# Suaiba/Mammo-CLIP-Dissect

Measured on AMD Instinct MI355X. Metric: probe images/sec dissected (763 concepts, all layers), higher is better.
Workload: dtype f32; 1 GPU; configs[1]: M-Mammo-CLIP Dissect through the drop-in driver describe_broad_neurons.main(): Mammo-CLIP ViT-B/16 target+dissector (random init), weak: 10000 images per GPU, synthetic 224x224 images resident in HBM, 763 concepts, 12 layers x 768 neurons, soft_wpmi top_k=100; CSV + args.txt + activation cache files written inside the step; entry_point=mammo_clip_dissect_amd.concept_vit.describe_broad_neurons.main, images_per_gpu=10000, global_images=10000, batch=2500, parallelism=image-sharded dp1, activation_cache_written=True

## Files before the change

### mammo-clip-dissect_amd/_lib.py

```python
import ctypes
import os

_HERE = os.path.dirname(os.path.abspath(__file__))
LIB_PATH = os.environ.get("MCD_LIB_PATH") or os.path.join(_HERE, "csrc", "libmcd_hip.so")

_i64 = ctypes.c_int64
_int = ctypes.c_int
_f = ctypes.c_float
_p = ctypes.c_void_p
_sz = ctypes.c_size_t

SIGNATURES = {
    "mcd_last_error": (ctypes.c_char_p, []),
    "mcd_abi_version": (_int, []),
    "mcd_normalize_rows": (_int, [_p, _i64, _i64, _i64, _p, _i64, _p]),
    "mcd_center_cube_normalize_rows": (_int, [_p, _i64, _i64, _i64, _f, _p, _i64, _p]),
    "mcd_prepare_rows_gathered": (_int, [_p, _i64, _i64, _int, ctypes.POINTER(_i64), _i64, _i64, _i64, _int, _f, _p, _i64,
                                         _p]),
    "mcd_embed_gemm_workspace": (_sz, [_i64, _i64, _i64, _int]),
    "mcd_embed_gemm": (_int, [_p, _i64, _p, _i64, _i64, _i64, _i64, _int, _p, _i64, _p, _sz, _p]),
    "mcd_embed_gemm_exp_workspace": (_sz, [_i64, _i64, _i64]),
    "mcd_embed_gemm_exp": (_int, [_p, _i64, _p, _i64, _i64, _i64, _i64, _f, _int, _p, _i64, _p, _p, _sz, _p]),
    "mcd_embed_gemm_exp_time_kernel": (_int, [_int]),
    "mcd_embed_gemm_exp_kernel_ms": (_f, []),
# ... 22 lines not shown
    "mcd_conv7x7s2_nhwc": (_int, [_p, _i64, _i64, _i64, _i64, _p, _i64, _p, _p]),
    "mcd_bn_relu_maxpool_nhwc": (_int, [_p, _i64, _i64, _i64, _i64, _p, _p, _p, _p]),
    "mcd_conv_igemm_nhwc": (_int, [_p, _i64, _i64, _i64, _i64, _p, _p, _i64, _int, _int, _int, _int, _p, _p]),
    "mcd_conv_igemm_res_nhwc": (_int, [_p, _i64, _i64, _i64, _i64, _p, _p, _p, _i64, _int, _int, _int, _int, _p, _p]),
    "mcd_conv3x3s2_nhwc": (_int, [_p, _i64, _i64, _i64, _i64, _p, _p, _i64, _int, _p, _p]),
    "mcd_avgpool2_nhwc": (_int, [_p, _i64, _i64, _i64, _i64, _p, _p]),
    "mcd_attnpool_tokens": (_int, [_p, _i64, _i64, _i64, _p, _p, _p]),
    "mcd_image_preprocess": (_int, [_p, _i64, _i64, _i64, _p, _i64, _i64, _p, _i64, _i64, _i64, _i64, _i64, _i64, _p, _p, _i64,
                                    _p]),
    "mcd_image_minmax_workspace": (_sz, [_i64, _i64, _i64, _i64]),
    "mcd_image_minmax_normalize": (_int, [_p, _i64, _i64, _i64, _i64, _int, _f, _f, _p, _i64, _p, _sz, _p]),
}
TEXT_SIGNATURES = {
    "mcd_vit_attention_keylen": (_int, [_p, _i64, _i64, _i64, _p, _p, _p]),
    "mcd_text_embed_ln": (_int, [_p, _p, _p, _p, _p, _p, _p, _f, _i64, _i64, _i64, _i64, _i64, _p, _p]),
}
CLIP_SIGNATURES = {
    "mcd_vit_attention_causal": (_int, [_p, _i64, _i64, _i64, _p, _p]),
    "mcd_quick_gelu": (_int, [_p, _i64, _p, _p]),
}
TOKEN_SIGNATURES = {
    "mcd_token_mean": (_int, [_p, _int, _int, _int, _i64, _i64, _int, _p, _i64, _p]),
}

MCD_E_ARG = -1
MCD_E_RANGE = -2
MCD_E_WORKSPACE = -3
MCD_E_UNSUPPORTED = -5

_lib = None


class McdError(RuntimeError):

    def __init__(self, code, msg):
        super().__init__(msg)
        self.code = code


def load():
    global _lib
    if _lib is None:
        if not os.path.exists(LIB_PATH):
            raise ImportError(
                "mammo-clip-dissect_amd: %s not found. Build it with `python -c 'import __graft_entry__ as g; "
                "g.build()'` or `make -C mammo-clip-dissect_amd/csrc`. There is no CPU fallback." % LIB_PATH)
        L = ctypes.CDLL(LIB_PATH)
        for name, (res, args) in (list(SIGNATURES.items()) + list(TEXT_SIGNATURES.items()) + list(CLIP_SIGNATURES.items())
                                  + list(TOKEN_SIGNATURES.items())):
            fn = getattr(L, name)
            fn.restype = res
            fn.argtypes = args
        _lib = L
    return _lib


def check(rc):
    if rc != 0:
        msg = load().mcd_last_error().decode("utf-8", "replace")
        raise McdError(rc, msg)


BLASLT_PATH = os.path.join(os.path.dirname(LIB_PATH), "libmcd_blaslt.so")
BLASLT_SIGNATURES = {
    "mcd_blaslt_last_error": (ctypes.c_char_p, []),
    "mcd_linear_residual_workspace": (_sz, []),
    "mcd_linear_residual": (_int, [_p, _i64, _p, _i64, _p, _p, _i64, _p, _i64, _i64, _i64, _i64, _p, _sz, _p]),
    "mcd_linear_residual_relu": (_int, [_p, _i64, _p, _i64, _p, _p, _i64, _p, _i64, _i64, _i64, _i64, _p, _sz, _p]),
    "mcd_linear_residual_plan_info": (_int, [_i64, _i64, _i64, ctypes.POINTER(_f), ctypes.POINTER(_int)]),
    "mcd_linear_residual_get_picks": (_int, [ctypes.POINTER(_i64), _int]),
    "mcd_linear_residual_set_pick": (_int, [_i64, _i64, _i64, _int, _int]),
}
_blaslt = None


def load_blaslt():
    global _blaslt
    if _blaslt is None:
        try:
            L = ctypes.CDLL(BLASLT_PATH)
            for name, (res, args) in BLASLT_SIGNATURES.items():
                fn = getattr(L, name)
                fn.restype = res
                fn.argtypes = args
            _blaslt = L
        except (OSError, AttributeError):
            _blaslt = False
    return _blaslt or None
```

### mammo-clip-dissect_amd/concept_vit/utils.py

```python
import os
import re
import threading

import torch
from torch.utils.data import DataLoader

from .. import core
from ..pipeline import Dissector
from . import data_utils

PM_SUFFIX = {"max": "_max", "avg": ""}
_P_CACHE = {}


def get_activation(outputs, mode):
    if mode not in ("avg", "max"):
        raise ValueError("pool mode must be 'avg' or 'max'")

    def hook(model, input, output):
        if mode == 'avg' and type(output) is tuple:
            output = output[0]
        out = output.detach()
        if out.dim() not in (2, 3, 4):
            return
# ... 44 lines not shown
        words = (f.read()).split('\n')
    return [i for i in words if i != ""]


def _layer_widths(model, layers, sample, forward):
    cache = model.__dict__.setdefault("_mcd_layer_widths", {})
    missing = [m for m in layers if id(m) not in cache]
    if missing:
        got = {}
        hs = [m.register_forward_hook(lambda mod, i, o, k=id(m): got.__setitem__(k, o[0] if type(o) is tuple else o))
              for m in missing]
        with torch.no_grad():
            forward(sample)
        for h in hs:
            h.remove()
        for m in missing:
            o = got[id(m)]
            cache[id(m)] = int(o.shape[1] if o.dim() in (2, 4) else o.shape[2])
    return [cache[id(m)] for m in layers]


class Extraction:

    def __init__(self, dis, E_txt, target_layers, writer=None):
        self.dis, self.E_txt, self.target_layers, self.writer = dis, E_txt, list(target_layers), writer

    def start_writer(self):
        if self.writer is not None and not self.writer.is_alive() and not self.writer.started:
            self.writer.begin()

    def wait(self):
        if self.writer is not None:
            self.start_writer()
            self.writer.join()
            if self.writer.error is not None:
                raise self.writer.error
            self.writer = None


class _CacheWriter(threading.Thread):

    def __init__(self, device, jobs):
        super().__init__(daemon=True)
        self.device, self.jobs, self.error, self.started = device, jobs, None, False
        self.ready = None

    def begin(self):
        self.started = True
        if torch.device(self.device).type == "cuda":
            with torch.cuda.device(self.device):
                self.ready = torch.cuda.Event()
                self.ready.record()
        self.start()

    def _save_some(self, items):
        try:
            for t, path in items:
                torch.save(t, path)
        except Exception as e:
            self.error = e
# ... 59 lines not shown
            E_txt = torch.cat(feats)
            if write_caches:
                torch.save(E_txt.cpu(), text_save_name)
        if not (need_target or need_clip):
            return None
        if E_txt is None:
            E_txt = _load_feats(text_save_name, device)
        N = len(dataset)
        on_device = hasattr(dataset, "device_batches") and getattr(dataset, "device", None) is not None
        if on_device:
            batches = dataset.device_batches(batch_size)
            first = (dataset.sample() if hasattr(dataset, "sample") else dataset.images()[:1]) if N > 0 else None
        else:
            batches = DataLoader(dataset, batch_size=batch_size, shuffle=False, num_workers=0)
            first = _views(dataset[0][0])[0].unsqueeze(0).to(device) if N > 0 else None
        if first is None:
            first = torch.zeros((1, 3, 224, 224), dtype=torch.float32, device=device)
        layers = [resolve_layer(target_model, l) for l in target_layers]
        widths = _layer_widths(target_model, layers, first, encode_target)
        same = target_model is clip_model
        dis = Dissector(N, list(target_layers), widths, len(words), E_txt.shape[1], device,
                        pool_mode=pool_mode, gather=gather)
        handles = [m.register_forward_hook(dis.hook(i)) for i, m in enumerate(layers)] if need_target else []
        try:
            for batch in batches:
                if not on_device:
                    batch = batch[0] if isinstance(batch, (list, tuple)) else batch["images"]
                target_view, clip_view = _views(batch)
                images = target_view.to(device)
                clip_images = images if clip_view is target_view else clip_view.to(device)
                if need_target:
                    out = encode_target(images)
                if need_clip:
                    if same and need_target and clip_images is images:
                        f = out
                    else:
                        f = clip_model.encode_image(clip_images)
                    if getattr(clip_model, "projection", False):
                        f = clip_model.image_projection(f)
                    dis.add_image_features(f.float())
                dis.advance(images.shape[0])
        finally:
            for h in handles:
                h.remove()
        if not need_clip:
            dis.E_img.copy_(_load_feats(clip_save_name, device))
        if not need_target:
            for i, l in enumerate(target_layers):
                A = torch.load(layer_files[l], map_location='cpu', weights_only=True).float().to(device)
                core.transpose(A, out=dis.At[dis.offsets[i]:dis.offsets[i + 1], :N])
        writer = None
        if write_caches:
            jobs = []
            if need_clip:
                jobs.append((lambda: dis.E_img, clip_save_name))
            if need_target:
                for i, l in enumerate(target_layers):
                    jobs.append((lambda i=i: dis.At[dis.offsets[i]:dis.offsets[i + 1], :N].t(), layer_files[l]))
            writer = _CacheWriter(device, jobs)
        return Extraction(dis, E_txt, target_layers, writer)


def _views(batch):
    if isinstance(batch, (list, tuple)):
        target, clip = batch
        return target, clip
    return batch, batch


def _probe_data(d_probe, device, preprocess=None, clip_preprocess=None):
    from ..pipeline import shard_bounds
    world, rank = _dist_info()
    n = len(data_utils.get_data(d_probe, None))
    lo, hi = shard_bounds(n, world, rank)
# ... 65 lines not shown
```

### mammo-clip-dissect_amd/core.py

```python
import ctypes
import functools

import torch

from . import _lib
from ._lib import McdError, check

POOL_MODES = {"avg": 0, "max": 1, "cls": 2, "none": 3}
POOL_SILU_AVG = 4
GEMM_MODES = {"f32": 0, "bf16x3": 1, "bf16": 2}


def _stream():
    return ctypes.c_void_p(torch.cuda.current_stream().cuda_stream)


def _on_device(fn):
    @functools.wraps(fn)
    def wrapper(*args, **kw):
        dev = None
        for a in list(args) + list(kw.values()):
            if isinstance(a, torch.Tensor) and a.is_cuda:
                if dev is None:
                    dev = a.device
# ... 755 lines not shown
    if out is None:
        out = torch.empty(h.shape[:-1] + (N,), dtype=torch.float32, device=h.device)
    elif tuple(out.shape) != tuple(h.shape[:-1]) + (N,):
        raise ValueError("linear_residual: out has shape %s" % (tuple(out.shape),))
    ws = _blaslt_ws.get(h.device)
    if ws is None:
        ws = _blaslt_ws[h.device] = torch.empty((L.mcd_linear_residual_workspace(),), dtype=torch.uint8, device=h.device)
    ev = LINEAR_EVENTS
    if ev is not None:
        e0, e1 = torch.cuda.Event(enable_timing=True), torch.cuda.Event(enable_timing=True)
        e0.record()
    fn = L.mcd_linear_residual_relu if relu else L.mcd_linear_residual
    rc = fn(h.data_ptr(), ldh, weight.data_ptr(), K, bias.data_ptr() if bias is not None else None,
            res.data_ptr() if res is not None else None, ldr, out.data_ptr(), N, M, N, K, ws.data_ptr(), ws.numel(), _stream())
    if ev is not None:
        e1.record()
        ev.append((e0, e1, M, N, K))
    if rc != 0:
        raise _lib.McdError(rc, L.mcd_blaslt_last_error().decode("utf-8", "replace"))
    return out


@_on_device
def hook_pool(x, mode, dst, row0, col0, neuron_major):
    _need_gpu(x, dst)
    if x.dtype != torch.float32:
        x = x.float()
    nhwc = mode in ("avg", "max") and channels_last(x, only=True)
    if not nhwc:
        x = x.contiguous()
    if x.dim() == 4:
        B, Cout, HW = x.shape[0], x.shape[1], x.shape[2] * x.shape[3]
        m = POOL_MODES[mode]
    elif x.dim() == 3:
        B, HW, Cout = x.shape
        m = POOL_MODES["cls"]
    elif x.dim() == 2:
        B, Cout = x.shape
        HW = 1
        m = POOL_MODES["none"]
    else:
        raise ValueError("unsupported hook output shape %s" % (tuple(x.shape),))
    if dst.dtype != torch.float32 or dst.dim() != 2 or dst.stride(1) != 1:
        raise TypeError("dst must be a 2-D float32 matrix with unit inner stride")
    need = (col0 + Cout, row0 + B) if neuron_major else (row0 + B, col0 + Cout)
    if row0 < 0 or col0 < 0 or dst.shape[0] < need[0] or dst.shape[1] < need[1]:
        raise IndexError("hook_pool: block [%d:%d, %d:%d] outside the activation matrix %s"
                         % (row0, row0 + B, col0, col0 + Cout, tuple(dst.shape)))
    if neuron_major:
        sn, su = 1, dst.stride(0)
    else:
        sn, su = dst.stride(0), 1
    L = _lib.load()
    if nhwc:
        check(L.mcd_hook_pool_nhwc(x.data_ptr(), B, Cout, HW, m, dst.data_ptr(), int(row0), int(col0), sn, su, _stream()))
        return Cout
    check(L.mcd_hook_pool(x.data_ptr(), B, Cout, HW, m, dst.data_ptr(), int(row0), int(col0), sn, su, _stream()))
    return Cout


IMAGE_MAX_TAPS = 128
_PRECISION_BITS = 22
IMAGENET_MEAN, IMAGENET_STD = (0.485, 0.456, 0.406), (0.229, 0.224, 0.225)
CLIP_MEAN, CLIP_STD = (0.48145466, 0.4578275, 0.40821073), (0.26862954, 0.26130258, 0.27577711)


def _bilinear(x):
    x = -x if x < 0.0 else x
    return 1.0 - x if x < 1.0 else 0.0


def _bicubic(x):
    a = -0.5
    x = -x if x < 0.0 else x
    if x < 1.0:
        return ((a + 2.0) * x - (a + 3.0)) * x * x + 1
    if x < 2.0:
        return (((x - 5) * x + 8) * x - 4) * a
# ... 231 lines not shown
```

### mammo-clip-dissect_amd/csrc/k_pool.hip

```cpp
#include "mcd_common.h"

namespace {

template <bool VEC4>
__global__ __launch_bounds__(256) void pool_plane_kernel(const float* __restrict__ x, int64_t planes, int64_t Cout,
                                                          int64_t HW, int mode, float* __restrict__ dst, int64_t row0,
                                                          int64_t col0, int64_t stride_n, int64_t stride_u) {
    const int lane = threadIdx.x & 63;
    const int64_t plane = (int64_t)blockIdx.x * 4 + (threadIdx.x >> 6);
    if (plane >= planes) return;
    const float* src = x + plane * HW;
    float s = 0.f, m = -INFINITY;
    bool has_nan = false;
    if constexpr (VEC4) {
        const float4* s4 = reinterpret_cast<const float4*>(src);
        const int64_t n4 = HW >> 2;
        for (int64_t i = lane; i < n4; i += 64) {
            const float4 v = s4[i];
            s += (v.x + v.y) + (v.z + v.w);
            m = fmaxf(fmaxf(m, fmaxf(v.x, v.y)), fmaxf(v.z, v.w));
            has_nan |= (v.x != v.x) | (v.y != v.y) | (v.z != v.z) | (v.w != v.w);
        }
    } else {
        for (int64_t i = lane; i < HW; i += 64) {
            const float v = src[i];
            s += v;
            m = fmaxf(m, v);
            has_nan |= (v != v);
        }
    }
    s = mcd_wave_sum(s);
    m = mcd_wave_max(m);
    if (__ballot(has_nan)) m = __uint_as_float(0x7fc00000u);
    if (lane == 0) {
        const int64_t b = plane / Cout, ch = plane - b * Cout;
        dst[(row0 + b) * stride_n + (col0 + ch) * stride_u] = (mode == MCD_POOL_AVG) ? s / (float)HW : m;
    }
}

__global__ __launch_bounds__(256) void pool_copy_kernel(const float* __restrict__ x, int64_t B, int64_t F,
                                                         int64_t bstride, float* __restrict__ dst, int64_t row0,
                                                         int64_t col0, int64_t stride_n, int64_t stride_u) {
    const int64_t i = (int64_t)blockIdx.x * 256 + threadIdx.x;
    if (i >= B * F) return;
    const int64_t b = i / F, f = i - b * F;
    dst[(row0 + b) * stride_n + (col0 + f) * stride_u] = x[b * bstride + f];
}

}

extern "C" int mcd_hook_pool(const float* x, int64_t B, int64_t Cout, int64_t HW, int mode, float* dst, int64_t row0,
                             int64_t col0, int64_t stride_n, int64_t stride_u, mcd_stream_t stream) {
    MCD_REQUIRE(x && dst, MCD_E_ARG, "mcd_hook_pool: NULL pointer");
    MCD_REQUIRE(B >= 0 && Cout > 0 && HW > 0 && row0 >= 0 && col0 >= 0, MCD_E_ARG, "mcd_hook_pool: bad shape");
    MCD_REQUIRE(mode >= MCD_POOL_AVG && mode <= MCD_POOL_NONE, MCD_E_ARG, "mcd_hook_pool: bad mode %d", mode);
    if (B == 0) return MCD_OK;
    hipStream_t st = (hipStream_t)stream;
    if (mode == MCD_POOL_AVG || mode == MCD_POOL_MAX) {
        const int64_t planes = B * Cout;
        const unsigned grid = (unsigned)mcd_cdiv(planes, 4);
        const bool vec4 = (HW % 4 == 0) && (((uintptr_t)x) % 16 == 0);
        if (vec4)
            hipLaunchKernelGGL(pool_plane_kernel<true>, dim3(grid), dim3(256), 0, st, x, planes, Cout, HW, mode, dst,
                               row0, col0, stride_n, stride_u);
        else
            hipLaunchKernelGGL(pool_plane_kernel<false>, dim3(grid), dim3(256), 0, st, x, planes, Cout, HW, mode, dst,
                               row0, col0, stride_n, stride_u);
        MCD_LAUNCH_CHECK("pool_plane_kernel");
    } else {
        const int64_t bstride = (mode == MCD_POOL_CLS) ? HW * Cout : Cout;
        const unsigned grid = (unsigned)mcd_cdiv(B * Cout, 256);
        hipLaunchKernelGGL(pool_copy_kernel, dim3(grid), dim3(256), 0, st, x, B, Cout, bstride, dst, row0, col0,
                           stride_n, stride_u);
        MCD_LAUNCH_CHECK("pool_copy_kernel");
    }
    return MCD_OK;
}
```

### mammo-clip-dissect_amd/csrc/mcd_host.c

```c
#include <math.h>
#include <stdint.h>
#include <string.h>

static const double P10[9] = {1.0, 1e1, 1e2, 1e3, 1e4, 1e5, 1e6, 1e7, 1e8};
static const uint64_t I10[9] = {1ull, 10ull, 100ull, 1000ull, 10000ull, 100000ull, 1000000ull, 10000000ull, 100000000ull};

static int ndigits(uint64_t v) {
    int n = 1;
    while (v >= 10) { v /= 10; ++n; }
    return n;
}

static void shortest(float v, uint64_t* ip, uint64_t* fp, int* dp) {
    const float av = fabsf(v);
    const double x = (double)av;
    const double hi = (x + (double)nextafterf(av, INFINITY)) * 0.5, lo = (x + (double)nextafterf(av, 0.0f)) * 0.5;
    int d = 0, low = 0, high = 0;
    double y = 0, fl = 0;
    for (;; ++d) {
        y = x * P10[d];
        fl = floor(y);
        low = fl > lo * P10[d];
        high = fl + 1.0 < hi * P10[d];
        if (low || high || d == 8) break;
    }
// ... 142 lines not shown
            *e++ = '[';
            for (int j = 0; j < k; ++j) {
                const int32_t w = ids[r * k + j];
                if (w < 0 || w >= n_words) return -1;
                if (j) { *e++ = ','; *e++ = ' '; }
                memcpy(e, reprs[w], (size_t)repr_lens[w]);
                e += repr_lens[w];
            }
            *e++ = ']';
            o = emit_field(o, d, e - d);
        }
        *o++ = ',';
        int n = mcd_fmt_f32_row(vals + r * k, k, cell, (int)sizeof(cell));
        if (n < 0) return -1;
        o = emit_field(o, cell, n);
        *o++ = ',';
        n = mcd_fmt_i64_row(imgs + r * k_img, k_img, cell, (int)sizeof(cell));
        if (n < 0) return -1;
        o = emit_field(o, cell, n);
        *o++ = '\n';
    }
    return (int64_t)(o - out);
}
```

### mammo-clip-dissect_amd/pipeline.py

```python
import os

import torch
import torch.distributed as dist

from . import _lib
from . import core as _hip_ops


STAGE_MARK = None

ROW_FNS = ("rank_reorder", "cos_similarity", "cos_similarity_cubed")


def _round_up(x, m):
    return (x + m - 1) // m * m


def shard_align():
    try:
        return max(1, int(os.environ.get("MCD_SHARD_ALIGN", "1")))
    except ValueError:
        return 1


# ... 56 lines not shown
        if self.world > 1:
            mine = torch.tensor([[self.n_local]], dtype=torch.int64, device=self.device)
            self.counts = [int(v) for v in self._gather(mine).view(-1).tolist()]
        else:
            self.counts = [self.n_local]
        self.n_total = sum(self.counts)
        self.n_max = max(self.counts)
        self.row0 = sum(self.counts[:self.rank])
        self.layer_names = list(layer_names)
        self.layer_widths = [int(w) for w in layer_widths]
        self.offsets = [0]
        for w in self.layer_widths:
            self.offsets.append(self.offsets[-1] + w)
        self.U = self.offsets[-1]
        self.C, self.D = int(n_concepts), int(embed_dim)
        self.pool_mode = pool_mode
        self.gemm_mode = gemm_mode
        self.set_scoring(similarity_fn, None if similarity_fn in ROW_FNS else top_k, a=a, lam=lam, min_prob=min_prob,
                         p_start=p_start, p_end=p_end)
        self.ldA = _round_up(max(self.n_local, 1), 64)
        self.At = torch.zeros((self.U, self.ldA), dtype=torch.float32, device=self.device)
        self.E_img = torch.zeros((self.n_local, self.D), dtype=torch.float32, device=self.device)
        self.cursor = 0

    def set_scoring(self, similarity_fn="soft_wpmi", top_k=None, a=None, lam=None, min_prob=1e-7, p_start=0.998,
                    p_end=0.97, p=3, top_fraction=0.05, scale_p=0.5, min_norm=1e-3):
        if similarity_fn in ROW_FNS:
            if top_k is not None:
                raise TypeError("%s() got an unexpected keyword argument 'top_k'" % similarity_fn)
            if self.gemm_mode == "bf16":
                raise NotImplementedError("gemm_mode='bf16' never materialises fp32 P, which %s scores: use 'f32', "
                                          "'bf16x3' or 'bf16_p'" % similarity_fn)
            self.similarity_fn = similarity_fn
            self.top_k = 0
            self.rr_p, self.top_fraction, self.scale_p = float(p), float(top_fraction), float(scale_p)
            self.min_norm = float(min_norm)
            return
        if similarity_fn not in ("soft_wpmi", "wpmi"):
            raise NotImplementedError("fused pipeline supports soft_wpmi, wpmi, %s (got %r)" % (", ".join(ROW_FNS),
                                                                                             similarity_fn))
        self.similarity_fn = similarity_fn
        soft = similarity_fn == "soft_wpmi"
        self.top_k = int(top_k if top_k is not None else (100 if soft else 28))
        self.a = float(a if a is not None else (10 if soft else 2))
        self.lam = lam if lam is not None else (1 if soft else 0.6)
        self.min_prob = float(min_prob)
        self.p = None
        self.p_ok = True
        if soft:
            self.p = (p_start - (torch.arange(start=0, end=self.top_k) / self.top_k * (p_start - p_end))).float().to(
                self.device)
            self.p_ok = 0.0 <= min(p_start, p_end) and max(p_start, p_end) <= 1.0

    def reset(self):
        self.cursor = 0

    def hook(self, layer_index):
        col0 = self.offsets[layer_index]
        width = self.layer_widths[layer_index]

        def _hook(module, inputs, output):
            if type(output) is tuple:
                output = output[0]
            n = self.ops.hook_pool(output.detach(), self.pool_mode, self.At, self.cursor, col0, True)
            if n != width:
                raise RuntimeError("layer %s produced %d neurons, expected %d" % (self.layer_names[layer_index], n, width))
        _hook.token0_only = True
        return _hook

    def add_image_features(self, feats):
        B = feats.shape[0]
        self.E_img[self.cursor:self.cursor + B].copy_(feats)

    def advance(self, batch):
        self.cursor += int(batch)
        if self.cursor > self.n_local:
            raise RuntimeError("more images than the dissector was sized for")

    def _all_gather_rows(self, t):
        if self.world == 1:
            return t
        return self._gather(t.contiguous())

    def _all_gather_ragged(self, t, lens):
        if self.world == 1:
            return t[:lens[0]]
        m = max(lens)
        mine = lens[self.rank]
        if t.shape[0] != m:
            pad = torch.zeros((m,) + tuple(t.shape[1:]), dtype=t.dtype, device=t.device)
            pad[:mine] = t[:mine]
            t = pad
        full = self._gather(t.contiguous())
        if all(n == m for n in lens):
            return full
        return torch.cat([full[r * m:r * m + lens[r]] for r in range(self.world)], dim=0)

    def _col_topk_global(self, K, mark):
        ops, G, N_l = self.ops, self.world, self.n_local
        Kl = min(K, N_l)
# ... 397 lines not shown
```

Before: 3979 images/s.

## Stream activation cache rows to disk during extraction via pinned slots and host writer

Adds a cache-streaming path. The pooling hook also writes each batch's pooled rows into a row-major staging block, which is pushed through a slot ring to host code. That code writes the rows straight into a torch.save placeholder zip at the tensor record's offset, computes the CRC incrementally and patches it in at close. This is meant to remove the end-of-extraction transpose, torch.save and file write work by overlapping it with the forward passes. The cost is extra staging memory, per-batch reserve and push synchronisation, and reliance on the torch.save zip layout; it is limited to single-process runs.

```diff
diff --git a/include/mcd_cache.h b/include/mcd_cache.h
--- /dev/null
+++ b/include/mcd_cache.h
@@ -0,0 +1,43 @@
+#ifndef MCD_CACHE_H
+#define MCD_CACHE_H
+
+#include <stddef.h>
+#include <stdint.h>
+
+#include "mcd_hip.h"
+
+#ifdef __cplusplus
+extern "C" {
+#endif
+
+int mcd_hook_pool_rows(const float* x, int64_t B, int64_t Cout, int64_t HW, int mode, float* dst, int64_t row0,
+                       int64_t col0, int64_t stride_n, int64_t stride_u, float* rows, int64_t width,
+                       mcd_stream_t stream);
+
+typedef struct {
+    int (*append)(void* file, const float* rows, int64_t row0, int64_t n);
+    int (*close)(void* file);
+    void (*abort)(void* file);
+    const char* (*last_error)(void);
+} mcd_cache_io_t;
+
+int mcd_cache_stream_open(int n_files, void* const* files, const int64_t* widths, const mcd_cache_io_t* io, int n_slots,
+                          size_t slot_bytes, void** handle);
+int mcd_cache_stream_reserve(void* handle, int file, mcd_stream_t stream);
+int mcd_cache_stream_push(void* handle, int file, const float* device_block, int64_t row0, int64_t n,
+                          mcd_stream_t stream);
+int mcd_cache_stream_close(void* handle);
+int mcd_cache_stream_abort(void* handle);
+
+uint32_t mcd_zip_crc32(uint32_t crc, const void* buf, size_t n);
+int mcd_cachefile_open(const char* part_path, const char* final_path, int64_t n_rows, int64_t width, int64_t data_off,
+                       int64_t crc_off_a, int64_t crc_off_b, void** out);
+int mcd_cachefile_append(void* file, const float* rows, int64_t row0, int64_t n);
+int mcd_cachefile_close(void* file);
+void mcd_cachefile_abort(void* file);
+const char* mcd_cachefile_last_error(void);
+
+#ifdef __cplusplus
+}
+#endif
+#endif
diff --git a/mammo-clip-dissect_amd/_lib.py b/mammo-clip-dissect_amd/_lib.py
--- a/mammo-clip-dissect_amd/_lib.py
+++ b/mammo-clip-dissect_amd/_lib.py
@@ -68,6 +68,15 @@
 TOKEN_SIGNATURES = {
     "mcd_token_mean": (_int, [_p, _int, _int, _int, _i64, _i64, _int, _p, _i64, _p]),
 }
+_pp = ctypes.POINTER(_p)
+CACHE_SIGNATURES = {
+    "mcd_hook_pool_rows": (_int, [_p, _i64, _i64, _i64, _int, _p, _i64, _i64, _i64, _i64, _p, _i64, _p]),
+    "mcd_cache_stream_open": (_int, [_int, _pp, ctypes.POINTER(_i64), _p, _int, _sz, _pp]),
+    "mcd_cache_stream_reserve": (_int, [_p, _int, _p]),
+    "mcd_cache_stream_push": (_int, [_p, _int, _p, _i64, _i64, _p]),
+    "mcd_cache_stream_close": (_int, [_p]),
+    "mcd_cache_stream_abort": (_int, [_p]),
+}
 
 MCD_E_ARG = -1
 MCD_E_RANGE = -2
@@ -93,7 +102,7 @@
                 "g.build()'` or `make -C mammo-clip-dissect_amd/csrc`. There is no CPU fallback." % LIB_PATH)
         L = ctypes.CDLL(LIB_PATH)
         for name, (res, args) in (list(SIGNATURES.items()) + list(TEXT_SIGNATURES.items()) + list(CLIP_SIGNATURES.items())
-                                  + list(TOKEN_SIGNATURES.items())):
+                                  + list(TOKEN_SIGNATURES.items()) + list(CACHE_SIGNATURES.items())):
             fn = getattr(L, name)
             fn.restype = res
             fn.argtypes = args
@@ -133,3 +142,38 @@
         except (OSError, AttributeError):
             _blaslt = False
     return _blaslt or None
+
+
+HOST_PATH = os.path.join(_HERE, "csrc", "libmcd_host.so")
+CACHE_HOST_SIGNATURES = {
+    "mcd_zip_crc32": (ctypes.c_uint32, [ctypes.c_uint32, _p, _sz]),
+    "mcd_cachefile_open": (_int, [ctypes.c_char_p, ctypes.c_char_p, _i64, _i64, _i64, _i64, _i64, _pp]),
+    "mcd_cachefile_append": (_int, [_p, _p, _i64, _i64]),
+    "mcd_cachefile_close": (_int, [_p]),
+    "mcd_cachefile_abort": (None, [_p]),
+    "mcd_cachefile_last_error": (ctypes.c_char_p, []),
+}
+_cache_host = None
+
+
+class CacheIO(ctypes.Structure):
+    _fields_ = [("append", _p), ("close", _p), ("abort", _p), ("last_error", _p)]
+
+
+def load_cache_host():
+    global _cache_host
+    if _cache_host is None:
+        try:
+            L = ctypes.CDLL(HOST_PATH)
+            for name, (res, args) in CACHE_HOST_SIGNATURES.items():
+                fn = getattr(L, name)
+                fn.restype = res
+                fn.argtypes = args
+            _cache_host = L
+        except (OSError, AttributeError):
+            _cache_host = False
+    return _cache_host or None
+
+
+def cache_io(H):
+    return CacheIO(*[ctypes.cast(getattr(H, "mcd_cachefile_" + n), _p) for n in ("append", "close", "abort", "last_error")])
diff --git a/mammo-clip-dissect_amd/concept_vit/utils.py b/mammo-clip-dissect_amd/concept_vit/utils.py
--- a/mammo-clip-dissect_amd/concept_vit/utils.py
+++ b/mammo-clip-dissect_amd/concept_vit/utils.py
@@ -90,20 +90,170 @@
 
 class Extraction:
 
-    def __init__(self, dis, E_txt, target_layers, writer=None):
+    def __init__(self, dis, E_txt, target_layers, writer=None, stream=None):
         self.dis, self.E_txt, self.target_layers, self.writer = dis, E_txt, list(target_layers), writer
+        self.stream = stream
 
     def start_writer(self):
         if self.writer is not None and not self.writer.is_alive() and not self.writer.started:
             self.writer.begin()
 
     def wait(self):
+        if self.stream is not None:
+            stream, self.stream = self.stream, None
+            stream.close()
         if self.writer is not None:
             self.start_writer()
             self.writer.join()
             if self.writer.error is not None:
                 raise self.writer.error
             self.writer = None
+
+
+CACHE_STREAM_SLOTS = 8
+
+
+def _placeholder_archive(part_path, n_rows, width):
+    import struct
+    import zipfile
+    torch.save(torch.empty((n_rows, width), dtype=torch.float32), part_path)
+    nbytes = n_rows * width * 4
+    with zipfile.ZipFile(part_path) as z:
+        recs = [i for i in z.infolist() if i.filename.endswith("/data/0")]
+        start_dir = z.start_dir
+    with open(part_path, "rb") as f:
+        def at(off, n):
+            f.seek(off)
+            return f.read(n)
+        ok = len(recs) == 1 and recs[0].compress_type == zipfile.ZIP_STORED and recs[0].file_size == nbytes
+        if ok:
+            zi = recs[0]
+            head = at(zi.header_offset, 30)
+            ok = head[:4] == b"PK\x03\x04"
+        if ok:
+            n_name, n_extra = struct.unpack("<HH", head[26:30])
+            data_off = zi.header_offset + 30 + n_name + n_extra
+            if zi.flag_bits & 0x8:
+                crc_b = data_off + nbytes + (4 if at(data_off + nbytes, 4) == b"PK\x07\x08" else 0)
+            else:
+                crc_b = zi.header_offset + 14
+            crc_a, pos = None, start_dir
+            while crc_a is None:
+                ent = at(pos, 46)
+                if len(ent) < 46 or ent[:4] != b"PK\x01\x02":
+                    break
+                n_name, n_extra, n_comment = struct.unpack("<HHH", ent[28:34])
+                if at(pos + 46, n_name) == zi.orig_filename.encode("utf-8"):
+                    crc_a = pos + 16
+                pos += 46 + n_name + n_extra + n_comment
+            want = struct.pack("<I", zi.CRC)
+            ok = crc_a is not None and at(crc_a, 4) == want and at(crc_b, 4) == want
+    if not ok:
+        os.unlink(part_path)
+        raise RuntimeError("torch.save wrote an archive whose tensor record was not found where the zip format puts it: %s "
+                           "(MCD_CACHE_STREAM=0 writes the cache files without the streaming route)" % part_path)
+    return data_off, crc_a, crc_b
+
+
+class CacheStream:
+
+    def __init__(self, device, n_rows, files, batch_rows, slots=None):
+        d = torch.device(device)
+        self.device = torch.device("cuda", d.index if d.index is not None else torch.cuda.current_device())
+        self.n_rows, self.files = int(n_rows), list(files)
+        self.slots = int(slots if slots is not None else CACHE_STREAM_SLOTS)
+        self.slot_bytes = max(4, int(batch_rows) * max(w for _, w in self.files) * 4)
+        self.handle, self.pending, self.closed, self.keep = None, [], False, {}
+        self.L, self.H = core._lib.load(), core._lib.load_cache_host()
+
+    def begin(self):
+        if self.handle is not None or self.closed:
+            return
+        import ctypes
+        H, n = self.H, len(self.files)
+        handles = (ctypes.c_void_p * n)()
+        try:
+            for i, (path, width) in enumerate(self.files):
+                part = path + ".part"
+                data_off, crc_a, crc_b = _placeholder_archive(part, self.n_rows, width)
+                h = ctypes.c_void_p()
+                if H.mcd_cachefile_open(os.fsencode(part), os.fsencode(path), self.n_rows, width, data_off, crc_a, crc_b,
+                                        ctypes.byref(h)) != 0:
+                    raise OSError(H.mcd_cachefile_last_error().decode("utf-8", "replace"))
+                handles[i] = h
+        except BaseException:
+            self.closed = True
+            for h in handles:
+                if h:
+                    H.mcd_cachefile_abort(h)
+            raise
+        widths = (ctypes.c_int64 * n)(*[w for _, w in self.files])
+        io = core._lib.cache_io(H)
+        out = ctypes.c_void_p()
+        with torch.cuda.device(self.device):
+            rc = self.L.mcd_cache_stream_open(n, handles, widths, ctypes.byref(io), self.slots, self.slot_bytes, ctypes.byref(out))
+        if rc != 0:
+            self.closed = True
+            core.check(rc)
+        self.handle = out
+        pending, self.pending = self.pending, []
+        if pending:
+            with torch.cuda.device(self.device):
+                self._side = torch.cuda.Stream(device=self.device)
+                for file, block, row0, n, ready in pending:
+                    self._side.wait_event(ready)
+                    with torch.cuda.stream(self._side):
+                        self.push(file, block, row0, n)
+
+    def reserve(self, file):
+        if self.handle is not None:
+            with torch.cuda.device(self.device):
+                core.check(self.L.mcd_cache_stream_reserve(self.handle, file, core._stream()))
+
+    def push(self, file, block, row0, n):
+        if self.closed:
+            raise RuntimeError("CacheStream is closed")
+        if block.dtype != torch.float32 or not block.is_contiguous() or block.dim() != 2 or block.shape[0] < n \
+                or block.shape[1] != self.files[file][1] or block.device != self.device:
+            raise TypeError("CacheStream.push: block must be contiguous float32 [>= %d, %d] on %s" % (n, self.files[file][1], self.device))
+        if self.handle is None:
+            with torch.cuda.device(self.device):
+                ready = torch.cuda.Event()
+                ready.record()
+            self.pending.append((file, block, row0, n, ready))
+            return
+        self.keep[file] = block
+        with torch.cuda.device(self.device):
+            core.check(self.L.mcd_cache_stream_push(self.handle, file, block.data_ptr(), int(row0), int(n), core._stream()))
+
+    def _end(self, entry):
+        if self.closed:
+            return
+        self.closed = True
+        self.pending = []
+        if self.handle is not None:
+            handle, self.handle = self.handle, None
+            try:
+                core.check(entry(handle))
+            finally:
+                self.keep = {}
+
+    def close(self):
+        if not self.closed and self.handle is None:
+            self.begin()
+        self._end(self.L.mcd_cache_stream_close)
+
+    def abort(self):
+        try:
+            self._end(self.L.mcd_cache_stream_abort)
+        except core._lib.McdError:
+            pass
+
+    def __del__(self):
+        try:
+            self.abort()
+        except Exception:
+            pass
 
 
 class _CacheWriter(threading.Thread):
@@ -209,6 +359,14 @@
         dis = Dissector(N, list(target_layers), widths, len(words), E_txt.shape[1], device,
                         pool_mode=pool_mode, gather=gather)
         handles = [m.register_forward_hook(dis.hook(i)) for i, m in enumerate(layers)] if need_target else []
+        stream = None
+        if write_caches and need_target and N > 0 and torch.device(device).type == "cuda" \
+                and os.environ.get("MCD_CACHE_STREAM", "1") != "0" and core._lib.load_cache_host() is not None:
+            files = [(layer_files[l], w) for l, w in zip(target_layers, widths)]
+            if need_clip:
+                files.append((clip_save_name, int(E_txt.shape[1])))
+            stream = CacheStream(dis.device, N, files, batch_size)
+            dis.attach_cache_stream(stream, batch_size, image_file=len(files) - 1 if need_clip else None)
         try:
             for batch in batches:
                 if not on_device:
@@ -227,9 +385,14 @@
                         f = clip_model.image_projection(f)
                     dis.add_image_features(f.float())
                 dis.advance(images.shape[0])
+        except BaseException:
+            if stream is not None:
+                stream.abort()
+            raise
         finally:
             for h in handles:
                 h.remove()
+            dis.cache_stream = None
         if not need_clip:
             dis.E_img.copy_(_load_feats(clip_save_name, device))
         if not need_target:
@@ -237,6 +400,8 @@
                 A = torch.load(layer_files[l], map_location='cpu', weights_only=True).float().to(device)
                 core.transpose(A, out=dis.At[dis.offsets[i]:dis.offsets[i + 1], :N])
         writer = None
+        if stream is not None:
+            return Extraction(dis, E_txt, target_layers, stream=stream)
         if write_caches:
             jobs = []
             if need_clip:
diff --git a/mammo-clip-dissect_amd/core.py b/mammo-clip-dissect_amd/core.py
--- a/mammo-clip-dissect_amd/core.py
+++ b/mammo-clip-dissect_amd/core.py
@@ -801,8 +801,10 @@
 
 
 @_on_device
-def hook_pool(x, mode, dst, row0, col0, neuron_major):
+def hook_pool(x, mode, dst, row0, col0, neuron_major, rows=None):
     _need_gpu(x, dst)
+    if rows is not None:
+        _need_gpu(rows)
     if x.dtype != torch.float32:
         x = x.float()
     nhwc = mode in ("avg", "max") and channels_last(x, only=True)
@@ -830,9 +832,21 @@
         sn, su = 1, dst.stride(0)
     else:
         sn, su = dst.stride(0), 1
+    if rows is not None and (rows.dtype != torch.float32 or rows.dim() != 2 or not rows.is_contiguous()
+                             or rows.shape[0] < B or rows.shape[1] != Cout):
+        raise TypeError("rows must be a contiguous float32 [>= %d, %d] block" % (B, Cout))
     L = _lib.load()
     if nhwc:
         check(L.mcd_hook_pool_nhwc(x.data_ptr(), B, Cout, HW, m, dst.data_ptr(), int(row0), int(col0), sn, su, _stream()))
+        if rows is not None:
+            if not neuron_major:
+                raise TypeError("hook_pool: rows with a channels-last input needs a neuron-major dst")
+            if B > 0:
+                transpose(dst[col0:col0 + Cout, row0:row0 + B], out=rows[:B])
+        return Cout
+    if rows is not None:
+        check(L.mcd_hook_pool_rows(x.data_ptr(), B, Cout, HW, m, dst.data_ptr(), int(row0), int(col0), sn, su, rows.data_ptr(),
+                                   Cout, _stream()))
         return Cout
     check(L.mcd_hook_pool(x.data_ptr(), B, Cout, HW, m, dst.data_ptr(), int(row0), int(col0), sn, su, _stream()))
     return Cout
diff --git a/mammo-clip-dissect_amd/csrc/k_pool.hip b/mammo-clip-dissect_amd/csrc/k_pool.hip
--- a/mammo-clip-dissect_amd/csrc/k_pool.hip
+++ b/mammo-clip-dissect_amd/csrc/k_pool.hip
@@ -1,11 +1,13 @@
 #include "mcd_common.h"
+#include "../../include/mcd_cache.h"
 
 namespace {
 
-template <bool VEC4>
+template <bool VEC4, bool ROWS>
 __global__ __launch_bounds__(256) void pool_plane_kernel(const float* __restrict__ x, int64_t planes, int64_t Cout,
                                                           int64_t HW, int mode, float* __restrict__ dst, int64_t row0,
-                                                          int64_t col0, int64_t stride_n, int64_t stride_u) {
+                                                          int64_t col0, int64_t stride_n, int64_t stride_u,
+                                                          float* __restrict__ rows, int64_t width) {
     const int lane = threadIdx.x & 63;
     const int64_t plane = (int64_t)blockIdx.x * 4 + (threadIdx.x >> 6);
     if (plane >= planes) return;
@@ -34,26 +36,32 @@
     if (__ballot(has_nan)) m = __uint_as_float(0x7fc00000u);
     if (lane == 0) {
         const int64_t b = plane / Cout, ch = plane - b * Cout;
-        dst[(row0 + b) * stride_n + (col0 + ch) * stride_u] = (mode == MCD_POOL_AVG) ? s / (float)HW : m;
+        const float v = (mode == MCD_POOL_AVG) ? s / (float)HW : m;
+        dst[(row0 + b) * stride_n + (col0 + ch) * stride_u] = v;
+        if constexpr (ROWS) rows[b * width + ch] = v;
     }
 }
 
+template <bool ROWS>
 __global__ __launch_bounds__(256) void pool_copy_kernel(const float* __restrict__ x, int64_t B, int64_t F,
                                                          int64_t bstride, float* __restrict__ dst, int64_t row0,
-                                                         int64_t col0, int64_t stride_n, int64_t stride_u) {
+                                                         int64_t col0, int64_t stride_n, int64_t stride_u,
+                                                         float* __restrict__ rows, int64_t width) {
     const int64_t i = (int64_t)blockIdx.x * 256 + threadIdx.x;
     if (i >= B * F) return;
     const int64_t b = i / F, f = i - b * F;
-    dst[(row0 + b) * stride_n + (col0 + f) * stride_u] = x[b * bstride + f];
+    const float v = x[b * bstride + f];
+    dst[(row0 + b) * stride_n + (col0 + f) * stride_u] = v;
+    if constexpr (ROWS) rows[b * width + f] = v;
 }
 
-}
-
-extern "C" int mcd_hook_pool(const float* x, int64_t B, int64_t Cout, int64_t HW, int mode, float* dst, int64_t row0,
-                             int64_t col0, int64_t stride_n, int64_t stride_u, mcd_stream_t stream) {
-    MCD_REQUIRE(x && dst, MCD_E_ARG, "mcd_hook_pool: NULL pointer");
-    MCD_REQUIRE(B >= 0 && Cout > 0 && HW > 0 && row0 >= 0 && col0 >= 0, MCD_E_ARG, "mcd_hook_pool: bad shape");
-    MCD_REQUIRE(mode >= MCD_POOL_AVG && mode <= MCD_POOL_NONE, MCD_E_ARG, "mcd_hook_pool: bad mode %d", mode);
+template <bool ROWS>
+int hook_pool(const char* who, const float* x, int64_t B, int64_t Cout, int64_t HW, int mode, float* dst, int64_t row0,
+              int64_t col0, int64_t stride_n, int64_t stride_u, float* rows, int64_t width, mcd_stream_t stream) {
+    MCD_REQUIRE(x && dst, MCD_E_ARG, "%s: NULL pointer", who);
+    MCD_REQUIRE(B >= 0 && Cout > 0 && HW > 0 && row0 >= 0 && col0 >= 0, MCD_E_ARG, "%s: bad shape", who);
+    MCD_REQUIRE(mode >= MCD_POOL_AVG && mode <= MCD_POOL_NONE, MCD_E_ARG, "%s: bad mode %d", who, mode);
+    if (ROWS) MCD_REQUIRE(rows && width >= Cout, MCD_E_ARG, "%s: rows is NULL or width %lld < Cout", who, (long long)width);
     if (B == 0) return MCD_OK;
     hipStream_t st = (hipStream_t)stream;
     if (mode == MCD_POOL_AVG || mode == MCD_POOL_MAX) {
@@ -61,18 +69,31 @@
         const unsigned grid = (unsigned)mcd_cdiv(planes, 4);
         const bool vec4 = (HW % 4 == 0) && (((uintptr_t)x) % 16 == 0);
         if (vec4)
-            hipLaunchKernelGGL(pool_plane_kernel<true>, dim3(grid), dim3(256), 0, st, x, planes, Cout, HW, mode, dst,
-                               row0, col0, stride_n, stride_u);
+            hipLaunchKernelGGL((pool_plane_kernel<true, ROWS>), dim3(grid), dim3(256), 0, st, x, planes, Cout, HW, mode, dst,
+                               row0, col0, stride_n, stride_u, rows, width);
         else
-            hipLaunchKernelGGL(pool_plane_kernel<false>, dim3(grid), dim3(256), 0, st, x, planes, Cout, HW, mode, dst,
-                               row0, col0, stride_n, stride_u);
+            hipLaunchKernelGGL((pool_plane_kernel<false, ROWS>), dim3(grid), dim3(256), 0, st, x, planes, Cout, HW, mode, dst,
+                               row0, col0, stride_n, stride_u, rows, width);
         MCD_LAUNCH_CHECK("pool_plane_kernel");
     } else {
         const int64_t bstride = (mode == MCD_POOL_CLS) ? HW * Cout : Cout;
         const unsigned grid = (unsigned)mcd_cdiv(B * Cout, 256);
-        hipLaunchKernelGGL(pool_copy_kernel, dim3(grid), dim3(256), 0, st, x, B, Cout, bstride, dst, row0, col0,
-                           stride_n, stride_u);
+        hipLaunchKernelGGL(pool_copy_kernel<ROWS>, dim3(grid), dim3(256), 0, st, x, B, Cout, bstride, dst, row0, col0,
+                           stride_n, stride_u, rows, width);
         MCD_LAUNCH_CHECK("pool_copy_kernel");
     }
     return MCD_OK;
 }
+
+}
+
+extern "C" int mcd_hook_pool(const float* x, int64_t B, int64_t Cout, int64_t HW, int mode, float* dst, int64_t row0,
+                             int64_t col0, int64_t stride_n, int64_t stride_u, mcd_stream_t stream) {
+    return hook_pool<false>("mcd_hook_pool", x, B, Cout, HW, mode, dst, row0, col0, stride_n, stride_u, nullptr, 0, stream);
+}
+
+extern "C" int mcd_hook_pool_rows(const float* x, int64_t B, int64_t Cout, int64_t HW, int mode, float* dst, int64_t row0,
+                                  int64_t col0, int64_t stride_n, int64_t stride_u, float* rows, int64_t width,
+                                  mcd_stream_t stream) {
+    return hook_pool<true>("mcd_hook_pool_rows", x, B, Cout, HW, mode, dst, row0, col0, stride_n, stride_u, rows, width, stream);
+}
diff --git a/mammo-clip-dissect_amd/csrc/mcd_cache.hip b/mammo-clip-dissect_amd/csrc/mcd_cache.hip
--- /dev/null
+++ b/mammo-clip-dissect_amd/csrc/mcd_cache.hip
@@ -0,0 +1,255 @@
+#include <condition_variable>
+#include <deque>
+#include <mutex>
+#include <string>
+#include <thread>
+#include <vector>
+
+#include "mcd_common.h"
+#include "../../include/mcd_cache.h"
+
+namespace {
+
+struct Slot {
+    void* host = nullptr;
+    hipEvent_t done = nullptr;
+};
+
+struct Ring {
+    std::mutex mu;
+    std::vector<Slot> slots;
+    size_t slot_bytes = 0;
+    int device = -1;
+    bool lent = false;
+};
+Ring g_ring;
+
+struct Job {
+    int slot, file;
+    int64_t row0, n;
+};
+
+struct Writer {
+    int device = 0;
+    hipStream_t copy = nullptr;
+    hipEvent_t ready = nullptr;
+    std::vector<void*> files;
+    std::vector<int64_t> widths;
+    std::vector<hipEvent_t> file_done;
+    std::vector<char> file_pushed;
+    mcd_cache_io_t io{};
+    int n_slots = 0;
+    size_t slot_bytes = 0;
+
+    std::mutex mu;
+    std::condition_variable cv_job, cv_free;
+    std::deque<Job> jobs;
+    std::vector<int> free_slots;
+    bool stop = false;
+    int err = MCD_OK;
+    std::string err_text;
+    std::thread worker;
+
+    void fail(int code, const std::string& text) {
+        if (err == MCD_OK) {
+            err = code;
+            err_text = text;
+        }
+    }
+};
+
+void ring_release_storage(Ring& r) {
+    for (Slot& s : r.slots) {
+        if (s.done) (void)hipEventDestroy(s.done);
+        if (s.host) (void)hipHostFree(s.host);
+    }
+    r.slots.clear();
+    r.slot_bytes = 0;
+}
+
+int ring_borrow(int device, int n_slots, size_t slot_bytes) {
+    std::lock_guard<std::mutex> g(g_ring.mu);
+    MCD_REQUIRE(!g_ring.lent, MCD_E_UNSUPPORTED, "mcd_cache_stream_open: another stream writer of this process is still open");
+    if (g_ring.device != device || g_ring.slot_bytes < slot_bytes || (int)g_ring.slots.size() < n_slots) {
+        ring_release_storage(g_ring);
+        g_ring.device = device;
+        for (int i = 0; i < n_slots; ++i) {
+            Slot s;
+            hipError_t e = hipHostMalloc(&s.host, slot_bytes, hipHostMallocDefault);
+            if (e == hipSuccess) e = hipEventCreateWithFlags(&s.done, hipEventDisableTiming | hipEventBlockingSync);
+            if (e != hipSuccess) {
+                if (s.host) (void)hipHostFree(s.host);
+                ring_release_storage(g_ring);
+                return mcd_fail(MCD_E_LAUNCH, "mcd_cache_stream_open: pinned slot %d of %zu bytes: %s", i, slot_bytes, hipGetErrorString(e));
+            }
+            g_ring.slots.push_back(s);
+        }
+        g_ring.slot_bytes = slot_bytes;
+    }
+    g_ring.lent = true;
+    return MCD_OK;
+}
+
+void ring_return() {
+    std::lock_guard<std::mutex> g(g_ring.mu);
+    g_ring.lent = false;
+}
+
+void worker_main(Writer* w) {
+    (void)hipSetDevice(w->device);
+    for (;;) {
+        Job j;
+        {
+            std::unique_lock<std::mutex> lk(w->mu);
+            w->cv_job.wait(lk, [&] { return w->stop || !w->jobs.empty(); });
+            if (w->jobs.empty()) return;
+            j = w->jobs.front();
+            w->jobs.pop_front();
+        }
+        const Slot& s = g_ring.slots[(size_t)j.slot];
+        const hipError_t e = hipEventSynchronize(s.done);
+        bool ok;
+        {
+            std::lock_guard<std::mutex> g(w->mu);
+            if (e != hipSuccess) w->fail(MCD_E_LAUNCH, std::string("mcd_cache_stream: device -> host copy: ") + hipGetErrorString(e));
+            ok = w->err == MCD_OK;
+        }
+        if (ok && w->io.append(w->files[(size_t)j.file], (const float*)s.host, j.row0, j.n) != 0) {
+            const char* t = w->io.last_error ? w->io.last_error() : nullptr;
+            std::lock_guard<std::mutex> g(w->mu);
+            w->fail(MCD_E_UNSUPPORTED, std::string("mcd_cache_stream: append: ") + (t ? t : "failed"));
+        }
+        {
+            std::lock_guard<std::mutex> g(w->mu);
+            w->free_slots.push_back(j.slot);
+        }
+        w->cv_free.notify_one();
+    }
+}
+
+void writer_destroy(Writer* w) {
+    for (hipEvent_t e : w->file_done)
+        if (e) (void)hipEventDestroy(e);
+    if (w->ready) (void)hipEventDestroy(w->ready);
+    if (w->copy) (void)hipStreamDestroy(w->copy);
+    delete w;
+}
+
+int writer_end(void* handle, bool commit, const char* who) {
+    Writer* w = (Writer*)handle;
+    MCD_REQUIRE(w, MCD_E_ARG, "%s: NULL handle", who);
+    {
+        std::lock_guard<std::mutex> g(w->mu);
+        w->stop = true;
+    }
+    w->cv_job.notify_one();
+    if (w->worker.joinable()) w->worker.join();
+    ring_return();
+    for (void* f : w->files) {
+        if (commit && w->err == MCD_OK) {
+            if (w->io.close(f) != 0) {
+                const char* t = w->io.last_error ? w->io.last_error() : nullptr;
+                w->fail(MCD_E_UNSUPPORTED, std::string("mcd_cache_stream_close: ") + (t ? t : "finalisation failed"));
+            }
+        } else {
+            w->io.abort(f);
+        }
+    }
+    const int err = w->err;
+    const std::string text = w->err_text;
+    writer_destroy(w);
+    return err == MCD_OK ? MCD_OK : mcd_fail(err, "%s", text.c_str());
+}
+
+}
+
+extern "C" int mcd_cache_stream_open(int n_files, void* const* files, const int64_t* widths, const mcd_cache_io_t* io, int n_slots,
+                                     size_t slot_bytes, void** handle) {
+    MCD_REQUIRE(handle, MCD_E_ARG, "mcd_cache_stream_open: NULL handle pointer");
+    *handle = nullptr;
+    const bool io_ok = io && io->append && io->close && io->abort;
+    bool args_ok = io_ok && n_files >= 1 && files && widths && n_slots >= 1 && n_slots <= 1024 && slot_bytes >= 4;
+    for (int i = 0; args_ok && i < n_files; ++i) args_ok = files[i] != nullptr && widths[i] > 0;
+    if (!args_ok) {
+        if (io_ok && files)
+            for (int i = 0; i < n_files; ++i)
+                if (files[i]) io->abort(files[i]);
+        return mcd_fail(MCD_E_ARG, "mcd_cache_stream_open: bad argument");
+    }
+    Writer* w = new Writer;
+    w->files.assign(files, files + n_files);
+    w->widths.assign(widths, widths + n_files);
+    w->io = *io;
+    w->file_done.assign((size_t)n_files, nullptr);
+    w->file_pushed.assign((size_t)n_files, 0);
+    w->n_slots = n_slots;
+    w->slot_bytes = slot_bytes;
+    hipError_t e = hipGetDevice(&w->device);
+    if (e == hipSuccess) e = hipStreamCreateWithFlags(&w->copy, hipStreamNonBlocking);
+    if (e == hipSuccess) e = hipEventCreateWithFlags(&w->ready, hipEventDisableTiming);
+    for (int i = 0; e == hipSuccess && i < n_files; ++i) e = hipEventCreateWithFlags(&w->file_done[(size_t)i], hipEventDisableTiming);
+    int rc = e == hipSuccess ? MCD_OK : mcd_fail(MCD_E_LAUNCH, "mcd_cache_stream_open: %s", hipGetErrorString(e));
+    if (rc == MCD_OK) rc = ring_borrow(w->device, n_slots, slot_bytes);
+    if (rc != MCD_OK) {
+        for (void* f : w->files) w->io.abort(f);
+        writer_destroy(w);
+        return rc;
+    }
+    for (int i = 0; i < n_slots; ++i) w->free_slots.push_back(i);
+    w->worker = std::thread(worker_main, w);
+    *handle = w;
+    return MCD_OK;
+}
+
+extern "C" int mcd_cache_stream_reserve(void* handle, int file, mcd_stream_t stream) {
+    Writer* w = (Writer*)handle;
+    MCD_REQUIRE(w && file >= 0 && file < (int)w->files.size(), MCD_E_ARG, "mcd_cache_stream_reserve: bad handle or file %d", file);
+    if (!w->file_pushed[(size_t)file]) return MCD_OK;
+    const hipError_t e = hipStreamWaitEvent((hipStream_t)stream, w->file_done[(size_t)file], 0);
+    MCD_REQUIRE(e == hipSuccess, MCD_E_LAUNCH, "mcd_cache_stream_reserve: %s", hipGetErrorString(e));
+    return MCD_OK;
+}
+
+extern "C" int mcd_cache_stream_push(void* handle, int file, const float* device_block, int64_t row0, int64_t n,
+                                     mcd_stream_t stream) {
+    Writer* w = (Writer*)handle;
+    MCD_REQUIRE(w && file >= 0 && file < (int)w->files.size(), MCD_E_ARG, "mcd_cache_stream_push: bad handle or file %d", file);
+    MCD_REQUIRE(row0 >= 0 && n >= 0, MCD_E_ARG, "mcd_cache_stream_push: bad rows");
+    if (n == 0) return MCD_OK;
+    MCD_REQUIRE(device_block, MCD_E_ARG, "mcd_cache_stream_push: NULL block");
+    const int64_t width = w->widths[(size_t)file];
+    MCD_REQUIRE((uint64_t)n <= w->slot_bytes / 4 / (uint64_t)width, MCD_E_ARG,
+                "mcd_cache_stream_push: %lld rows of %lld floats do not fit a slot of %zu bytes", (long long)n, (long long)width, w->slot_bytes);
+    const size_t bytes = (size_t)n * (size_t)width * 4;
+    int slot;
+    {
+        std::unique_lock<std::mutex> lk(w->mu);
+        w->cv_free.wait(lk, [&] { return !w->free_slots.empty(); });
+        slot = w->free_slots.back();
+        w->free_slots.pop_back();
+    }
+    const Slot& s = g_ring.slots[(size_t)slot];
+    hipError_t e = hipEventRecord(w->ready, (hipStream_t)stream);
+    if (e == hipSuccess) e = hipStreamWaitEvent(w->copy, w->ready, 0);
+    if (e == hipSuccess) e = hipMemcpyAsync(s.host, device_block, bytes, hipMemcpyDeviceToHost, w->copy);
+    if (e == hipSuccess) e = hipEventRecord(s.done, w->copy);
+    if (e == hipSuccess) e = hipEventRecord(w->file_done[(size_t)file], w->copy);
+    if (e != hipSuccess) {
+        (void)hipStreamSynchronize(w->copy);
+        std::lock_guard<std::mutex> g(w->mu);
+        w->free_slots.push_back(slot);
+        w->fail(MCD_E_LAUNCH, std::string("mcd_cache_stream_push: ") + hipGetErrorString(e));
+        return mcd_fail(MCD_E_LAUNCH, "mcd_cache_stream_push: %s", hipGetErrorString(e));
+    }
+    w->file_pushed[(size_t)file] = 1;
+    {
+        std::lock_guard<std::mutex> g(w->mu);
+        w->jobs.push_back(Job{slot, file, row0, n});
+    }
+    w->cv_job.notify_one();
+    return MCD_OK;
+}
+
+extern "C" int mcd_cache_stream_close(void* handle) { return writer_end(handle, true, "mcd_cache_stream_close"); }
+
+extern "C" int mcd_cache_stream_abort(void* handle) { return writer_end(handle, false, "mcd_cache_stream_abort"); }
diff --git a/mammo-clip-dissect_amd/csrc/mcd_host.c b/mammo-clip-dissect_amd/csrc/mcd_host.c
--- a/mammo-clip-dissect_amd/csrc/mcd_host.c
+++ b/mammo-clip-dissect_amd/csrc/mcd_host.c
@@ -1,6 +1,12 @@
+#define _POSIX_C_SOURCE 200809L
+#include <errno.h>
+#include <fcntl.h>
 #include <math.h>
 #include <stdint.h>
+#include <stdio.h>
+#include <stdlib.h>
 #include <string.h>
+#include <unistd.h>
 
 static const double P10[9] = {1.0, 1e1, 1e2, 1e3, 1e4, 1e5, 1e6, 1e7, 1e8};
 static const uint64_t I10[9] = {1ull, 10ull, 100ull, 1000ull, 10000ull, 100000ull, 1000000ull, 10000000ull, 100000000ull};
@@ -189,3 +195,156 @@
     }
     return (int64_t)(o - out);
 }
+
+static _Thread_local char g_cache_err[512];
+
+const char* mcd_cachefile_last_error(void) { return g_cache_err; }
+
+static int cache_fail(const char* what, const char* path, int err) {
+    if (err)
+        snprintf(g_cache_err, sizeof g_cache_err, "%s: %s: %s", what, path ? path : "", strerror(err));
+    else
+        snprintf(g_cache_err, sizeof g_cache_err, "%s: %s", what, path ? path : "");
+    return -1;
+}
+
+static uint32_t g_crc_tab[8][256];
+static int g_crc_ready;
+
+static void crc_init(void) {
+    for (uint32_t i = 0; i < 256; ++i) {
+        uint32_t c = i;
+        for (int k = 0; k < 8; ++k) c = (c & 1u) ? 0xEDB88320u ^ (c >> 1) : c >> 1;
+        g_crc_tab[0][i] = c;
+    }
+    for (uint32_t i = 0; i < 256; ++i)
+        for (int t = 1; t < 8; ++t) g_crc_tab[t][i] = (g_crc_tab[t - 1][i] >> 8) ^ g_crc_tab[0][g_crc_tab[t - 1][i] & 0xffu];
+    __atomic_store_n(&g_crc_ready, 1, __ATOMIC_RELEASE);
+}
+
+uint32_t mcd_zip_crc32(uint32_t crc, const void* buf, size_t n) {
+    const unsigned char* p = (const unsigned char*)buf;
+    if (!__atomic_load_n(&g_crc_ready, __ATOMIC_ACQUIRE)) crc_init();
+    uint32_t c = ~crc;
+    while (n && ((uintptr_t)p & 7u)) { c = g_crc_tab[0][(c ^ *p++) & 0xffu] ^ (c >> 8); --n; }
+    while (n >= 8) {
+        uint32_t lo, hi;
+        memcpy(&lo, p, 4);
+        memcpy(&hi, p + 4, 4);
+        lo ^= c;
+        c = g_crc_tab[7][lo & 0xffu] ^ g_crc_tab[6][(lo >> 8) & 0xffu] ^ g_crc_tab[5][(lo >> 16) & 0xffu] ^ g_crc_tab[4][lo >> 24] ^
+            g_crc_tab[3][hi & 0xffu] ^ g_crc_tab[2][(hi >> 8) & 0xffu] ^ g_crc_tab[1][(hi >> 16) & 0xffu] ^ g_crc_tab[0][hi >> 24];
+        p += 8;
+        n -= 8;
+    }
+    while (n--) c = g_crc_tab[0][(c ^ *p++) & 0xffu] ^ (c >> 8);
+    return ~c;
+}
+
+typedef struct {
+    int fd;
+    int64_t n_rows, width, rows_done, data_off, crc_off[2];
+    uint32_t crc;
+    char *part, *final;
+} mcd_cachefile;
+
+static int write_all(int fd, const void* buf, size_t n, int64_t off) {
+    const char* p = (const char*)buf;
+    while (n) {
+        const ssize_t w = pwrite(fd, p, n, (off_t)off);
+        if (w < 0) {
+            if (errno == EINTR) continue;
+            return -1;
+        }
+        p += w;
+        off += w;
+        n -= (size_t)w;
+    }
+    return 0;
+}
+
+static void cachefile_drop(mcd_cachefile* f, int unlink_part) {
+    if (f->fd >= 0) close(f->fd);
+    if (unlink_part && f->part) unlink(f->part);
+    free(f->part);
+    free(f->final);
+    free(f);
+}
+
+int mcd_cachefile_open(const char* part_path, const char* final_path, int64_t n_rows, int64_t width, int64_t data_off,
+                       int64_t crc_off_a, int64_t crc_off_b, void** out) {
+    if (!part_path || !final_path || !out) return cache_fail("mcd_cachefile_open", "NULL argument", 0);
+    *out = NULL;
+    if (n_rows < 0 || width <= 0 || data_off < 0 || crc_off_a < 0 || crc_off_b < 0 || n_rows > (INT64_MAX >> 3) / width)
+        return cache_fail("mcd_cachefile_open: bad shape or offset", part_path, 0);
+    const int64_t bytes = n_rows * width * 4, end = data_off + bytes;
+    const int64_t c[2] = {crc_off_a, crc_off_b};
+    for (int i = 0; i < 2; ++i)
+        if (c[i] + 4 > data_off && c[i] < end)
+            return cache_fail("mcd_cachefile_open: a CRC field lies inside the data record", part_path, 0);
+    mcd_cachefile* f = (mcd_cachefile*)calloc(1, sizeof *f);
+    if (!f) return cache_fail("mcd_cachefile_open: out of memory", part_path, 0);
+    f->fd = -1;
+    f->part = strdup(part_path);
+    f->final = strdup(final_path);
+    if (!f->part || !f->final) {
+        cachefile_drop(f, 0);
+        return cache_fail("mcd_cachefile_open: out of memory", part_path, 0);
+    }
+    f->fd = open(part_path, O_WRONLY | O_CLOEXEC);
+    if (f->fd < 0) {
+        const int e = errno;
+        cachefile_drop(f, 0);
+        return cache_fail("mcd_cachefile_open", part_path, e);
+    }
+    const off_t size = lseek(f->fd, 0, SEEK_END);
+    if (size < 0 || (int64_t)size < end || (int64_t)size < crc_off_a + 4 || (int64_t)size < crc_off_b + 4) {
+        cachefile_drop(f, 1);
+        return cache_fail("mcd_cachefile_open: the placeholder archive is shorter than its record", part_path, 0);
+    }
+    f->n_rows = n_rows;
+    f->width = width;
+    f->data_off = data_off;
+    f->crc_off[0] = crc_off_a;
+    f->crc_off[1] = crc_off_b;
+    *out = f;
+    return 0;
+}
+
+int mcd_cachefile_append(void* h, const float* rows, int64_t row0, int64_t n) {
+    mcd_cachefile* f = (mcd_cachefile*)h;
+    if (!f || n < 0 || (n > 0 && !rows)) return cache_fail("mcd_cachefile_append", "bad argument", 0);
+    if (row0 != f->rows_done) return cache_fail("mcd_cachefile_append: rows out of order", f->part, 0);
+    if (n > f->n_rows - f->rows_done) return cache_fail("mcd_cachefile_append: more rows than the file was opened for", f->part, 0);
+    const size_t bytes = (size_t)n * (size_t)f->width * 4;
+    if (write_all(f->fd, rows, bytes, f->data_off + f->rows_done * f->width * 4) != 0) return cache_fail("mcd_cachefile_append", f->part, errno);
+    f->crc = mcd_zip_crc32(f->crc, rows, bytes);
+    f->rows_done += n;
+    return 0;
+}
+
+void mcd_cachefile_abort(void* h) {
+    if (h) cachefile_drop((mcd_cachefile*)h, 1);
+}
+
+int mcd_cachefile_close(void* h) {
+    mcd_cachefile* f = (mcd_cachefile*)h;
+    if (!f) return cache_fail("mcd_cachefile_close", "NULL handle", 0);
+    int rc = 0;
+    if (f->rows_done != f->n_rows) {
+        snprintf(g_cache_err, sizeof g_cache_err, "mcd_cachefile_close: %s holds %lld of %lld rows", f->part,
+                 (long long)f->rows_done, (long long)f->n_rows);
+        rc = -1;
+    }
+    unsigned char le[4] = {(unsigned char)f->crc, (unsigned char)(f->crc >> 8), (unsigned char)(f->crc >> 16), (unsigned char)(f->crc >> 24)};
+    for (int i = 0; i < 2 && rc == 0; ++i)
+        if (write_all(f->fd, le, 4, f->crc_off[i]) != 0) rc = cache_fail("mcd_cachefile_close", f->part, errno);
+    if (rc == 0) {
+        const int fd = f->fd;
+        f->fd = -1;
+        if (close(fd) != 0) rc = cache_fail("mcd_cachefile_close", f->part, errno);
+    }
+    if (rc == 0 && rename(f->part, f->final) != 0) rc = cache_fail("mcd_cachefile_close: rename", f->final, errno);
+    cachefile_drop(f, rc != 0);
+    return rc;
+}
diff --git a/mammo-clip-dissect_amd/pipeline.py b/mammo-clip-dissect_amd/pipeline.py
--- a/mammo-clip-dissect_amd/pipeline.py
+++ b/mammo-clip-dissect_amd/pipeline.py
@@ -102,6 +102,13 @@
         self.At = torch.zeros((self.U, self.ldA), dtype=torch.float32, device=self.device)
         self.E_img = torch.zeros((self.n_local, self.D), dtype=torch.float32, device=self.device)
         self.cursor = 0
+        self.cache_stream = None
+
+    def attach_cache_stream(self, stream, batch_rows, image_file=None):
+        if self.world != 1:
+            raise RuntimeError("the activation-cache files are a single-process feature")
+        self.cache_stream, self._image_file = stream, image_file
+        self._stage = [torch.empty((int(batch_rows), w), dtype=torch.float32, device=self.device) for w in self.layer_widths]
 
     def set_scoring(self, similarity_fn="soft_wpmi", top_k=None, a=None, lam=None, min_prob=1e-7, p_start=0.998,
                     p_end=0.97, p=3, top_fraction=0.05, scale_p=0.5, min_norm=1e-3):
@@ -142,7 +149,17 @@
         def _hook(module, inputs, output):
             if type(output) is tuple:
                 output = output[0]
-            n = self.ops.hook_pool(output.detach(), self.pool_mode, self.At, self.cursor, col0, True)
+            out = output.detach()
+            if self.cache_stream is None:
+                n = self.ops.hook_pool(out, self.pool_mode, self.At, self.cursor, col0, True)
+            else:
+                stage, B = self._stage[layer_index], out.shape[0]
+                if B > stage.shape[0]:
+                    raise RuntimeError("layer %s handed the hook %d rows, the cache stream was sized for batches of %d"
+                                       % (self.layer_names[layer_index], B, stage.shape[0]))
+                self.cache_stream.reserve(layer_index)
+                n = self.ops.hook_pool(out, self.pool_mode, self.At, self.cursor, col0, True, rows=stage)
+                self.cache_stream.push(layer_index, stage, self.cursor, B)
             if n != width:
                 raise RuntimeError("layer %s produced %d neurons, expected %d" % (self.layer_names[layer_index], n, width))
         _hook.token0_only = True
@@ -151,11 +168,15 @@
     def add_image_features(self, feats):
         B = feats.shape[0]
         self.E_img[self.cursor:self.cursor + B].copy_(feats)
+        if self.cache_stream is not None and self._image_file is not None:
+            self.cache_stream.push(self._image_file, self.E_img[self.cursor:self.cursor + B], self.cursor, B)
 
     def advance(self, batch):
         self.cursor += int(batch)
         if self.cursor > self.n_local:
             raise RuntimeError("more images than the dissector was sized for")
+        if self.cache_stream is not None:
+            self.cache_stream.begin()
 
     def _all_gather_rows(self, t):
         if self.world == 1:
```

New measurement: 4042 images/s, median of 6. +1.6%, better.
